# rendeirolab/stainx

Measured on AMD Instinct MI355X. Metric: megapixels/sec Macenko transform, 64x3x512x512 fp32; max-abs vs torch CPU, higher is better.
Workload: dtype f32; 1 GPU; Macenko reference-mode transform, 64x3x512x512 fp32 per GPU (BASELINE configs[1]); tiles_per_gpu=64, height=512, width=512, input_batches_rotated=2, parallelism=tiles sharded over 1 GPU(s), no collective

## Files before the change

### stainx_amd/csrc/macenko.hip

```cpp
#include "common.hpp"

#include <algorithm>
#include <atomic>
#include <type_traits>
#include <cstdlib>

namespace sx {
namespace macenko {

constexpr int kSample = 4096;
constexpr int kMinCap = 8192;
constexpr int kChunk = 16384;
template <typename T> struct PackOf { static constexpr int n = 16 / (int)sizeof(T); };
constexpr int kSlots = 4;
constexpr int kMoments = 20;
constexpr int kPartial = 10;
constexpr int kShortList = 512;
constexpr int kGroupThreads = 1024;
constexpr int kKeys = kSample / kGroupThreads;
constexpr int kPrefetchHist = 8;
constexpr int kPrefetchCand = 8;
static_assert(kKeys * kGroupThreads == kSample && kPrefetchCand * kGroupThreads <= kMinCap, "per-tile stage geometry");

constexpr float kBeta = 0.15f;
// ... 49 lines not shown
    int recon_chunk, recon_blocks;
    int fast;
    int chunk;
    int vec_width;
    int no_tie;
    int out_code;
    int two_pass;
    int prior_units;
    unsigned prior_step_q16;
    uint32_t cap2;
    uint32_t seg_cap;
    uint32_t over_cap;
    int n_seg;
    int spec_fail;
    float spec_kw, spec_eff_far, spec_eff_near, spec_rot, spec_sigmas, spec_sigmas_conc, spec_tscale;
    int fused;
    int dense;
    uint32_t fused_cap;
    int fused_items;
    uint32_t code_epoch;
    const float* aug_alpha;
    const float* aug_beta;
    int own_basis;
};

static Geometry make_geometry(int64_t n_tiles, int64_t pixels, int pooled) {
    Geometry g{};
    g.n_tiles = n_tiles;
    g.pixels = pixels;
    g.blocks_per_tile = (int)((pixels + kChunk - 1) / kChunk);
    g.pooled = pooled;
    g.sample_stride = 1;
    g.cap = (uint32_t)kMinCap;
    g.chunk = kChunk;
    g.vec_width = 1;
    return g;
}

constexpr int kCompact = 32768;
struct alignas(256) PoolState {
    uint32_t hist[2][2][256];
    uint32_t below[kSlots], ncand[kSlots];
    uint32_t compact_n[kSlots];
    uint32_t rank_in_bin[kSlots], range[kSlots][2];
    uint32_t ok[kSlots], overflow;
    uint32_t status;
// ... 313 lines not shown
            return raw_value<T>(v);
        } else if constexpr (sizeof(T) == 4) {
            T v;
            __builtin_memcpy(&v, &w[k][e], 4);
            return raw_value<T>(v);
        } else {
            T v;
            __builtin_memcpy(&v, &w[k][2 * e], 8);
            return raw_value<T>(v);
        }
    }
};

template <int W>
__device__ __forceinline__ void store_codes(const Geometry& g, const Workspace& ws, int64_t tile, int64_t p, const uint32_t (&word)[3][W]) {
    static_assert(W == 1 || W == 2, "four or eight codes per plane");
#pragma unroll
    for (int c = 0; c < 3; ++c) {
        uint8_t* dst = ws.codes + ((size_t)tile * 3 + c) * g.pixels + p;
        if constexpr (W == 1) *reinterpret_cast<uint32_t*>(dst) = word[c][0]; else *reinterpret_cast<uint2*>(dst) = make_uint2(word[c][0], word[c][1]);
    }
}
template <typename T, int V, bool kInter, class Table>
__device__ __forceinline__ void code_quad(const PixelPacks<T, V, kInter>& u, int i0, const LevelTables<T>& tb, const Table& ct, const Geometry& g, const Workspace& ws, int64_t tile, float (&od_quad)[4][3], uint32_t (&word)[3][V / 4]) {
    static_assert((V == 4 || V == 8) && !kInter, "a pack's codes are one or two 32-bit words of a plane");
    constexpr int kCodeCopies = Table::copies;
    uint32_t differ = 0u;
    const int copy = (int)(threadIdx.x % kCodeCopies);
#pragma unroll
    for (int c = 0; c < 3; ++c) {
        uint32_t w = 0u;
#pragma unroll
        for (int ii = 0; ii < 4; ++ii) {
            const float x = u.value(c, i0 + ii);
            const uint32_t k = __float_as_uint(fmaf(x, 255.0f, 8388608.0f)) & 0xFFu;
            const uint2 entry = ct.e[k * kCodeCopies + copy];
            differ |= entry.x ^ __float_as_uint(x);
            od_quad[ii][c] = __uint_as_float(entry.y);
            w |= k << (8 * ii);
        }
        word[c][i0 / 4] = w;
    }
    if (__builtin_expect(__builtin_amdgcn_ballot_w64(differ != 0u) != 0ull, 0)) {
#pragma unroll
        for (int ii = 0; ii < 4; ++ii)
#pragma unroll
            for (int c = 0; c < 3; ++c) {
                float x = u.value(c, i0 + ii);
                asm volatile("" : "+v"(x));
                od_quad[ii][c] = od_of<T>(x, tb);
            }
        if (differ != 0u) put(&ws.code_bad[tile], g.code_epoch);
    }
}


template <typename O, int V, bool kInter>
__device__ __forceinline__ void store_pixels(O* __restrict__ dst, int64_t pixels, int64_t p, const O (&res)[3][V]) {
    if constexpr (kInter) {
        O flat[3][V];
#pragma unroll
        for (int i = 0; i < V; ++i)
#pragma unroll
            for (int c = 0; c < 3; ++c) flat[(3 * i + c) / V][(3 * i + c) % V] = res[c][i];
#pragma unroll
        for (int k = 0; k < 3; ++k) store_pack_stream<O, V>(dst + 3 * p + k * V, flat[k]);
    } else {
#pragma unroll
        for (int c = 0; c < 3; ++c) store_pack_stream<O, V>(dst + c * pixels + p, res[c]);
    }
}

template <typename O, int V>
__device__ __forceinline__ void store_pixels_staged(O* __restrict__ dst, int64_t p, const O (&res)[3][V], uint4* __restrict__ stage) {
    static_assert(sizeof(O) * V == 16, "16-byte packs");
    O flat[3][V];
// ... 2312 lines not shown
    hipLaunchKernelGGL((plane_kernel<T>), dim3(n_groups), dim3(kGroupThreads), 0, stream, images, g, ws, allow_fallback);
    hipLaunchKernelGGL((bracket_kernel<T, V, false, kInter>), dim3(grid_b), dim3(kStreamThreads), 0, stream, images, g, ws);
    if (g.spread) {
        hipLaunchKernelGGL(pool_reduce_kernel, dim3((unsigned)g.n_tiles), dim3(512), 0, stream, g, ws, 0);
        hipLaunchKernelGGL(pool_gather_kernel, dim3((unsigned)g.n_tiles), dim3(kGroupThreads), 0, stream, g, ws, 0);
        hipLaunchKernelGGL((stain_kernel<T, true>), dim3(1), dim3(kGroupThreads), 0, stream, images, g, ws);
    } else {
        hipLaunchKernelGGL((stain_kernel<T>), dim3(n_groups), dim3(kGroupThreads), 0, stream, images, g, ws);
    }
    if (g.own_basis) return check_launch("macenko estimate");
    hipLaunchKernelGGL((bracket_kernel<T, V, true, kInter>), dim3(grid_b), dim3(kStreamThreads), 0, stream, images, g, ws);
    if (g.spread) {
        hipLaunchKernelGGL(pool_reduce_kernel, dim3((unsigned)g.n_tiles), dim3(512), 0, stream, g, ws, 1);
        hipLaunchKernelGGL(pool_gather_kernel, dim3((unsigned)g.n_tiles), dim3(kGroupThreads), 0, stream, g, ws, 1);
        hipLaunchKernelGGL((scale_kernel<T, true>), dim3(1), dim3(kGroupThreads), 0, stream, images, g, ws, tmc, he_out, max_c_out);
    } else {
        hipLaunchKernelGGL((scale_kernel<T>), dim3(n_groups), dim3(kGroupThreads), 0, stream, images, g, ws, tmc, he_out, max_c_out);
    }
    return check_launch("macenko estimate");
}

template <typename T, int V, bool kInter = false>
static int run_two_pass(const T* images, const Geometry& g, const Workspace& ws, const float* tmc, hipStream_t stream, void* key_scratch = nullptr) {
    const unsigned n = (unsigned)g.n_tiles, grid = (unsigned)(g.n_tiles * g.blocks_per_tile);
#ifndef SX_DIAG
    if constexpr (V == 1) {
        return fail(SX_ERR_BAD_ARG, "the two-pass form needs 16-byte aligned tiles of whole packs");
    } else {
        if (!g.dense) return fail(SX_ERR_BAD_ARG, "the two-pass form serves tiles of up to 512 x 512 pixels in this build");
        hipLaunchKernelGGL((prior_kernel<T, true, kInter>), dim3(n), dim3(kGroupThreads), 0, stream, images, g, ws);
        hipLaunchKernelGGL((pass_a_kernel<T, V, kInter, true>), dim3(grid), dim3(kStreamThreads), 0, stream, images, g, ws);
        hipLaunchKernelGGL((estimate_stage_kernel<T, true>), dim3(2 * n), dim3(kGroupThreads), 0, stream, images, g, ws, tmc, static_cast<uint32_t*>(key_scratch));
        return check_launch("macenko two-pass estimate");
    }
#else
    const bool quads = (g.pixels % 4 == 0) && aligned_for(images, 4 * sizeof(T));
    if (quads)
        hipLaunchKernelGGL((prior_kernel<T, true, kInter>), dim3(n), dim3(kGroupThreads), 0, stream, images, g, ws);
    else
        hipLaunchKernelGGL((prior_kernel<T, false, kInter>), dim3(n), dim3(kGroupThreads), 0, stream, images, g, ws);
    if (g.dense) {
        hipLaunchKernelGGL((pass_a_kernel<T, V, kInter, true>), dim3(grid), dim3(kStreamThreads), 0, stream, images, g, ws);
        hipLaunchKernelGGL((estimate_stage_kernel<T, true>), dim3(2 * n), dim3(kGroupThreads), 0, stream, images, g, ws, tmc, static_cast<uint32_t*>(key_scratch));
    } else {
        hipLaunchKernelGGL((pass_a_kernel<T, V, kInter>), dim3(grid), dim3(kStreamThreads), 0, stream, images, g, ws);
        hipLaunchKernelGGL((estimate_stage_kernel<T>), dim3(2 * n), dim3(kGroupThreads), 0, stream, images, g, ws, tmc, static_cast<uint32_t*>(key_scratch));
    }
    return check_launch("macenko two-pass estimate");
#endif
}

#ifdef SX_DIAG
template <typename T, typename O, int V>
static int run_fused(const T* images, O* out, const Geometry& g, const Workspace& ws, const float* sm, const float* tmc, bool unit, hipStream_t stream) {
    const unsigned n = (unsigned)g.n_tiles, units = (unsigned)(2 * g.fused_items) + 2u * n;
    hipLaunchKernelGGL((prior_kernel<T, true, false>), dim3(n), dim3(kGroupThreads), 0, stream, images, g, ws);
    if (unit)
        hipLaunchKernelGGL((fused_kernel<T, O, V, true>), dim3(units), dim3(kStreamThreads), 0, stream, images, out, g, ws, sm, tmc);
    else
        hipLaunchKernelGGL((fused_kernel<T, O, V, false>), dim3(units), dim3(kStreamThreads), 0, stream, images, out, g, ws, sm, tmc);
    return check_launch("macenko fused transform");
// ... 17 lines not shown
    }
    if (rc != SX_OK) return rc;
    constexpr int VR = V == 1 ? 1 : ((int)(16 / sizeof(O)) < V ? (int)(16 / sizeof(O)) : V);
    Geometry gr = g;
    unsigned items_r = items;
    if (!g.recon_chunk && !g.fine_chunk && V > 1 && g.n_tiles * g.pixels >= (1ll << 22)) {
        gr.recon_chunk = kStreamThreads * VR;
        gr.recon_blocks = (int)((g.pixels + gr.recon_chunk - 1) / gr.recon_chunk);
        items_r = (unsigned)(g.n_tiles * gr.recon_blocks);
    }
    if (g.aug_alpha) {
        if (unit)
            hipLaunchKernelGGL((reconstruct_kernel<T, O, VR, true, kInter, true>), dim3(items_r), dim3(kStreamThreads), 0, stream, images, out, gr, ws, sm);
        else
            hipLaunchKernelGGL((reconstruct_kernel<T, O, VR, false, kInter, true>), dim3(items_r), dim3(kStreamThreads), 0, stream, images, out, gr, ws, sm);
    } else if (unit) {
        hipLaunchKernelGGL((reconstruct_kernel<T, O, VR, true, kInter>), dim3(items_r), dim3(kStreamThreads), 0, stream, images, out, gr, ws, sm);
    } else {
        hipLaunchKernelGGL((reconstruct_kernel<T, O, VR, false, kInter>), dim3(items_r), dim3(kStreamThreads), 0, stream, images, out, gr, ws, sm);
    }
    return check_launch("macenko reconstruct");
}

#ifdef SX_DIAG
static int device_cus() {
    static int cached[64] = {0};
    int dev = 0;
    if (hipGetDevice(&dev) != hipSuccess || dev < 0 || dev >= 64) return 256;
    if (cached[dev] == 0) {
        int n = 0;
        if (hipDeviceGetAttribute(&n, hipDeviceAttributeMultiprocessorCount, dev) != hipSuccess || n <= 0) n = 256;
        cached[dev] = n;
    }
    return cached[dev];
}
static int elem_bytes(int dtype) { return dtype == SX_U8 ? 1 : (dtype == SX_F16 || dtype == SX_BF16) ? 2 : dtype == SX_F32 ? 4 : 8; }
static bool resident_able(int dtype, int64_t n, int64_t pixels, unsigned flags) {
    if (dtype != SX_U8 && dtype != SX_F16 && dtype != SX_BF16 && dtype != SX_F32) return false;
    if (flags & (SX_MACENKO_SAMPLED | SX_MACENKO_CHANNELS_LAST | SX_MACENKO_OUT_BF16 | SX_MACENKO_OUT_F16)) return false;
    const int64_t pack = 16 / elem_bytes(dtype);
    if (pixels % pack != 0 || pixels < 1024) return false;
    const int64_t items = (pixels + kChunk - 1) / kChunk, group = (items + kResQuads - 1) / kResQuads;
    return group <= kResMaxGroup && group <= device_cus() && n >= 1;
}
static ResGeom resident_geometry(int dtype, int64_t n, int64_t pixels, bool unit) {
    Geometry g = make_geometry(n, pixels, 0);
    g.vec = 1;
    g.vec_width = 16 / elem_bytes(dtype);
    set_chunk(g, false);
    ResGeom rg{};
    rg.n_tiles = n;
    rg.pixels = pixels;
    rg.items = g.blocks_per_tile;
    rg.chunk = g.chunk;
    rg.group = (rg.items + kResQuads - 1) / kResQuads;
    const int cus = device_cus();
    int fit = std::max(cus / rg.group, 1);
    if (fit >= 8 && n >= 8) {
// ... 71 lines not shown
        g.spec_rot = kSpecRot;
        g.spec_sigmas = kSpecSigmas;
        g.spec_sigmas_conc = kSpecSigmasConc;
        g.spec_tscale = kSpecThresholdScale;
#ifdef SX_STAMPS
        auto knob = [](const char* name, float& v) { if (const char* e = std::getenv(name)) v = (float)std::atof(e); };
        knob("SX_SPEC_KW", g.spec_kw);
        knob("SX_SPEC_EFF_FAR", g.spec_eff_far);
        knob("SX_SPEC_EFF_NEAR", g.spec_eff_near);
        knob("SX_SPEC_ROT", g.spec_rot);
        knob("SX_SPEC_SIGMAS", g.spec_sigmas);
        knob("SX_SPEC_SIGMAS_CONC", g.spec_sigmas_conc);
        knob("SX_SPEC_TSCALE", g.spec_tscale);
#endif
        g.fused_cap = g.fused ? fused_cap_for(g.pixels) : dense_cap_for(g.pixels);
        g.fused_items = (int)(g.n_tiles * g.blocks_per_tile);
        g.cap2 = cap2_for(g.pixels);
        g.n_seg = even_items_size(g.pixels) ? g.blocks_per_tile * (kStreamThreads / kWave) : two_pass_segments(g.pixels);
        g.seg_cap = seg_cap_for(g.pixels);
        g.over_cap = over_cap_for(g.pixels);
        const int64_t n_sectors = g.pixels / 16;
        g.prior_units = (int)std::min<int64_t>(std::max<int64_t>(n_sectors / 4, std::min<int64_t>(n_sectors, 64)), kPriorUnitsMax);
        g.prior_step_q16 = (unsigned)((n_sectors << 16) / g.prior_units);
    }
    if (!g.fused) set_fine_chunk(g, vec ? W : 1);
#ifdef SX_STAMPS
    if (const char* e = std::getenv("SX_RECON_CHUNK")) {
        const int64_t c = std::atoll(e);
        if (c > 0 && !g.fused && c % ((int64_t)kStreamThreads * (vec ? W : 1)) == 0) {
            g.recon_chunk = (int)c;
            g.recon_blocks = (int)((g.pixels + c - 1) / c);
        }
    }
#endif
    const T* in = static_cast<const T*>(images);
    if constexpr (sizeof(T) == 1) {
        if (u8_half) {
#define SX_RUN_HALF(O)                                                                                                                                          \
    return g.interleaved ? (vec ? run_transform<T, O, W, true>(in, static_cast<O*>(out), g, ws, sm, tmc, unit, stream)                                          \
                                : run_transform<T, O, 1, true>(in, static_cast<O*>(out), g, ws, sm, tmc, unit, stream))                                         \
                         : (vec ? run_transform<T, O, W>(in, static_cast<O*>(out), g, ws, sm, tmc, unit, stream)                                                \
                                : run_transform<T, O, 1>(in, static_cast<O*>(out), g, ws, sm, tmc, unit, stream));
            if (g.out_code == SX_BF16) {
                SX_RUN_HALF(__hip_bfloat16)
            } else {
                SX_RUN_HALF(__half)
// ... 934 lines not shown
```

### stainx_amd/csrc/macenko_twopass.hpp

```cpp
#pragma once

namespace sx {
namespace macenko {

constexpr int kPriorSweeps = 4;
constexpr int kPriorUnitsMax = kGroupThreads / 4 * kPriorSweeps;
constexpr int kQueue2 = 512;
constexpr float kSpecSigmasConc = 5.0f, kSpecThresholdScale = 1.0f;
constexpr float kSpecSigmas = 5.0f;
constexpr float kSpecEffFar = 2.0f, kSpecEffNear = 1.0f;
__device__ __forceinline__ float spec_eff(const Geometry& g) { return g.prior_step_q16 >= (8u << 16) ? g.spec_eff_far : g.spec_eff_near; }
constexpr float kSpecKw = 0.10f, kSpecKx = 1.3e-3f;
constexpr float kSpecRot = 0.30f;
constexpr uint32_t kSpecSlow = 1u, kSpecHazard = 2u;
constexpr int kMaxSegments = 256;

constexpr int kRowBelowA = 0, kRowAboveA = 1, kRowBelowB = 2, kRowAboveB = 3, kRowConc = 4, kRowW = 8;
struct alignas(128) PriorRecord {
    float a0[3], a1[3], an[3];
    float rows[16][4];
    float kw, kx;
    float cmax[4];
    int32_t mode;
    int32_t min_first;
    uint32_t open;
};

struct alignas(64) FusedTile {
    uint32_t a_done;
    uint32_t s_done;
    uint32_t ncand[kSlots];
    uint32_t pad[10];
};
constexpr int kXcds = 8;
struct alignas(64) FusedQueue {
    uint32_t ticket;
    uint32_t pad[15];
};
struct FusedSched {
    FusedQueue queue[kXcds];
};
static_assert(sizeof(FusedTile) == kFusedTileBytes && sizeof(FusedSched) <= kFusedSchedBytes, "workspace layout");


typedef unsigned int sx_u4 __attribute__((ext_vector_type(4)));
__device__ __forceinline__ uint32_t ld_agent(const uint32_t* p) { return __hip_atomic_load(p, __ATOMIC_RELAXED, __HIP_MEMORY_SCOPE_AGENT); }
__device__ __forceinline__ int32_t ld_agent(const int32_t* p) { return __hip_atomic_load(p, __ATOMIC_RELAXED, __HIP_MEMORY_SCOPE_AGENT); }
__device__ __forceinline__ float ld_agent(const float* p) { return __uint_as_float(__hip_atomic_load(reinterpret_cast<const uint32_t*>(p), __ATOMIC_RELAXED, __HIP_MEMORY_SCOPE_AGENT)); }
__device__ __forceinline__ double ld_agent(const double* p) {
    return __longlong_as_double((long long)__hip_atomic_load(reinterpret_cast<const unsigned long long*>(p), __ATOMIC_RELAXED, __HIP_MEMORY_SCOPE_AGENT));
}
__device__ __forceinline__ void st_agent(uint32_t* p, uint32_t v) { __hip_atomic_store(p, v, __ATOMIC_RELAXED, __HIP_MEMORY_SCOPE_AGENT); }
__device__ __forceinline__ void st_agent(float* p, float v) { __hip_atomic_store(reinterpret_cast<uint32_t*>(p), __float_as_uint(v), __ATOMIC_RELAXED, __HIP_MEMORY_SCOPE_AGENT); }
__device__ __forceinline__ void st_agent(double* p, double v) {
    __hip_atomic_store(reinterpret_cast<unsigned long long*>(p), (unsigned long long)__double_as_longlong(v), __ATOMIC_RELAXED, __HIP_MEMORY_SCOPE_AGENT);
// ... 56 lines not shown
    const int64_t p = have ? ((int64_t)sector * 4 + (tid & 3)) * 4 : (int64_t)(tid & 3) * 4;
    if constexpr (kVec) {
        load_pixels<T, 4, kInter>(img, g.pixels, p, u);
    } else {
#pragma unroll
        for (int i = 0; i < 4; ++i) {
            float v[3][1];
            load_pixels<T, 1, kInter>(img, g.pixels, p + i, v);
#pragma unroll
            for (int c = 0; c < 3; ++c) u[c][i] = v[c][0];
        }
    }
    return have;
}
template <typename T>
__device__ __forceinline__ void prior_densities(const float (&u)[3][4], float (&od)[4][3]) {
#pragma unroll
    for (int i = 0; i < 4; ++i)
#pragma unroll
        for (int c = 0; c < 3; ++c) od[i][c] = optical_density<T>(u[c][i]);
}

template <typename T, bool kVec, bool kInter>
__global__ __launch_bounds__(kGroupThreads) void prior_kernel(const T* __restrict__ images, Geometry g, Workspace ws) {
    __shared__ PriorScratch sh;
    const int tile = blockIdx.x, tid = threadIdx.x, wave = tid / kWave;
    const uint32_t lane = lane_id();
    GroupState& st = ws.state[tile];
    PriorRecord* pr = &ws.prior[tile];
    const T* img = images + (int64_t)tile * 3 * g.pixels;
    SX_STAMP(st, 0);
    if (tid < kSlots) {
        put(&st.ncand[tid], 0u);
        put(&st.below[tid], 0u);
        put(&st.ncand_seen[tid], 0u);
        put(&st.over_count[tid], 0u);
    }
    if (tid < 2) put(&st.phi_pub[tid], 0ull);
    if ((g.fused || g.dense) && tid < (int)(sizeof(FusedTile) / 4)) put(reinterpret_cast<uint32_t*>(&ws.ftile[tile]) + tid, 0u);
    if (g.fused && tile == 0 && tid >= 32 && tid < 32 + kXcds) put(&ws.fsched->queue[tid - 32].ticket, 0u);
    if (tid == 0) {
        put(&st.fell_back, 0u);
        put(&st.spec, 0u);
        sh.n_kept = sh.n_all = sh.hazard = sh.open = sh.r_max = 0;
        sh.cmax[0] = sh.cmax[1] = sh.cmax[2] = sh.cmax[3] = 0;
    }
    for (int i = tid; i < 5 * kPriorBins; i += kGroupThreads) (&sh.hist[0][0])[i] = 0;

    {
        float m[kPartial];
#pragma unroll
        for (int k = 0; k < kPartial; ++k) m[k] = 0.0f;
        float raw[kPriorSweeps][3][4];
        bool have_quad[kPriorSweeps];
#pragma unroll
        for (int s = 0; s < kPriorSweeps; ++s) have_quad[s] = prior_fetch<T, kVec, kInter>(img, g, s, raw[s]);
#pragma unroll
        for (int s = 0; s < kPriorSweeps; ++s) {
            float od[4][3];
            prior_densities<T>(raw[s], od);
            const bool have = have_quad[s];
#pragma unroll
// ... 240 lines not shown
        }
        if (lane < 16 && (lane < (uint32_t)kRowConc || lane >= (uint32_t)kRowW)) {
#pragma unroll
            for (int c = 0; c < 4; ++c) put(&pr->rows[lane][c], __half2float(__float2half_rn(row[c])));
        }
    } else if (wave == 5 && lane == 0) {
#pragma unroll
        for (int i = 0; i < 3; ++i) {
            put(&pr->a0[i], sh.frame[i]);
            put(&pr->a1[i], sh.frame[3 + i]);
            put(&pr->an[i], sh.frame[6 + i]);
        }
        put(&pr->kw, g.spec_kw);
        put(&pr->kx, kSpecKx);
#pragma unroll
        for (int q = 0; q < 4; ++q) put(&pr->cmax[q], __uint_as_float(sh.cmax[q]));
        put(&pr->mode, 0);
        put(&pr->min_first, min_first ? 1 : 0);
        put(&pr->open, sh.open);
    }
    SX_STAMP(st, 7);
}

template <int TPB> struct PassAScratch {
    StatsScratch<TPB> stats;
    uint32_t queue[TPB / kWave][4][kQueue2];
    uint32_t below[2];
};

__device__ __forceinline__ void write_records(const uint32_t (*__restrict__ queue)[kQueue2], uint32_t n, uint32_t (&have)[kSlots], float* __restrict__ cand_tile, const Geometry& g, uint32_t seg_base, uint32_t* __restrict__ over_count) {
    const uint32_t cap2 = g.cap2, seg_cap = g.seg_cap, over_base = (uint32_t)g.n_seg * g.seg_cap;
    for (uint32_t i0 = 0; i0 < n; i0 += kWave) {
        const uint32_t i = i0 + lane_id();
        uint4 rec = make_uint4(0u, 0u, 0u, 0u);
        if (i < n) rec = make_uint4(queue[0][i], queue[1][i], queue[2][i], queue[3][i]);
#pragma unroll
        for (int s = 0; s < kSlots; ++s) {
            const bool has = ((rec.w >> s) & 1u) != 0;
            const uint64_t mask = __builtin_amdgcn_ballot_w64(has);
            const uint32_t count = (uint32_t)__popcll(mask), at = have[s] + rank_in_mask(mask);
            uint32_t idx = seg_base + at;
            bool store = has;
            if (__builtin_expect(have[s] + count > seg_cap, 0)) {
                const uint64_t spilled = __builtin_amdgcn_ballot_w64(has && at >= seg_cap);
                uint32_t base = 0;
                if (lane_id() == 0) base = atomicAdd(&over_count[s], (uint32_t)__popcll(spilled));
// ... 34 lines not shown
    for (int s = 0; s < kSlots; ++s) at0[s] = (uint32_t)__builtin_amdgcn_readlane((int)base, s);
    const auto rsrc = __builtin_amdgcn_make_buffer_rsrc(rec_tile, 0, (int)(kSlots * cap * 16u), 0x00020000);
    for (uint32_t i0 = 0; i0 < n; i0 += kWave) {
        const uint32_t i = i0 + lane;
        sx_u4 rec = {0u, 0u, 0u, 0u};
        uint32_t flags = 0;
        if (i < n) {
            rec[0] = queue[0][i];
            rec[1] = queue[1][i];
            rec[2] = queue[2][i];
            flags = queue[3][i];
        }
#pragma unroll
        for (int s = 0; s < kSlots; ++s) {
            const bool has = ((flags >> s) & 1u) != 0;
            const uint64_t mask = __builtin_amdgcn_ballot_w64(has);
            const uint32_t at = at0[s] + rank_in_mask(mask);
            if (has && at < cap) __builtin_amdgcn_raw_buffer_store_b128(rec, rsrc, (int)(((uint32_t)s * cap + at) * 16u), 0, 16);
            at0[s] += (uint32_t)__popcll(mask);
        }
    }
}

template <typename T, int V, int TPB, bool kInter, bool kFused = false, bool kEmit = false>
__device__ __forceinline__ void pass_a_item(const T* __restrict__ images, const Geometry& g, const Workspace& ws, int64_t tile, int chunk_id, int64_t item, PassAScratch<TPB>* sh, const LevelTables<T>& tb,
                                            const CodeTable<T, 2>* __restrict__ ct = nullptr) {
    const int64_t p_begin = (int64_t)chunk_id * g.chunk;
    const int64_t p_end = min(p_begin + (int64_t)g.chunk, g.pixels);
    const T* img = images + tile * 3 * g.pixels;
    GroupState& st = ws.state[tile];
    const PriorRecord* __restrict__ pr = &ws.prior[tile];
    const int wave = __builtin_amdgcn_readfirstlane((int)(threadIdx.x / kWave));
    const bool speculate = get(&pr->mode) == 0;
    typedef _Float16 half8 __attribute__((ext_vector_type(8)));
    typedef float float16v __attribute__((ext_vector_type(16)));
    half8 test_rows;
    {
        const uint32_t l = lane_id(), r = l & 31u, h = l >> 5, row_half = (r >> 2) & 1u, test = (r & 3u) + 4u * (r >> 3);
        const float4 coef = *reinterpret_cast<const float4*>(&pr->rows[test][0]);
        const bool mine = h == row_half;
        test_rows[0] = (_Float16)(mine ? coef.x : 0.0f);
        test_rows[1] = (_Float16)(mine ? coef.y : 0.0f);
        test_rows[2] = (_Float16)(mine ? coef.z : 0.0f);
        test_rows[3] = (_Float16)(mine ? coef.w : 0.0f);
        test_rows[4] = test_rows[5] = test_rows[6] = test_rows[7] = (_Float16)0.0f;
    }
    const float kw = get(&pr->kw), kx = get(&pr->kx);
    if (threadIdx.x < 2) sh->below[threadIdx.x] = 0;

    constexpr int kShortRun = 32 / V > 0 ? 32 / V : 1;
    double acc[kPartial];
#pragma unroll
    for (int k = 0; k < kPartial; ++k) acc[k] = 0.0;
    float m[kPartial];
#pragma unroll
    for (int k = 0; k < kPartial; ++k) m[k] = 0.0f;

    uint32_t (*queue)[kQueue2] = sh->queue[wave];
    uint32_t n_q = 0, have[kSlots] = {0u, 0u, 0u, 0u}, below_a = 0, below_b = 0;
    float* cand_tile = ws.cand_od + (size_t)tile * kSlots * 3 * g.cap2;
    const uint32_t seg = (uint32_t)chunk_id * (TPB / kWave) + (uint32_t)wave, seg_base = seg * g.seg_cap;
    auto flush = [&]() {
        if constexpr (kFused)
            write_records_fused(queue, n_q, ws.cand_rec + (size_t)tile * kSlots * g.fused_cap, g.fused_cap, ws.ftile[tile].ncand);
        else
            write_records(queue, n_q, have, cand_tile, g, seg_base, st.over_count);
        n_q = 0;
    };

// ... 29 lines not shown
                uint64_t valid[G];
                float16v forms[G];
#pragma unroll
                for (int gi = 0; gi < G; ++gi) {
#pragma unroll
                    for (int c = 0; c < 3; ++c) {
                        if constexpr (kEmit) od[gi][c] = od_quad[(i0 + gi) % 4][c]; else od[gi][c] = od_of<T>(u.value(c, i0 + gi), tb);
                    }
                    const bool sel = od_selected(od[gi], false);
                    valid[gi] = __builtin_amdgcn_ballot_w64(sel) & live_mask;
                    if (__builtin_amdgcn_inverse_ballot_w64(valid[gi])) {
                        const float* o = od[gi];
                        m[0] += 1.0f;
                        m[1] += o[0];
                        m[2] += o[1];
                        m[3] += o[2];
                        m[4] = fmaf(o[0], o[0], m[4]);
                        m[5] = fmaf(o[0], o[1], m[5]);
                        m[6] = fmaf(o[0], o[2], m[6]);
                        m[7] = fmaf(o[1], o[1], m[7]);
                        m[8] = fmaf(o[1], o[2], m[8]);
                        m[9] = fmaf(o[2], o[2], m[9]);
                    }
                    if constexpr (kTests) {
                        typedef __fp16 fp16x2 __attribute__((ext_vector_type(2)));
                        typedef uint32_t uint4v __attribute__((ext_vector_type(4)));
                        const fp16x2 p01 = __builtin_amdgcn_cvt_pkrtz(od[gi][0], od[gi][1]), p2c = __builtin_amdgcn_cvt_pkrtz(od[gi][2], 1.0f);
                        uint4v packed;
                        packed[0] = __builtin_bit_cast(uint32_t, p01);
                        packed[1] = __builtin_bit_cast(uint32_t, p2c);
                        packed[2] = packed[3] = 0u;
                        float16v zero;
#pragma unroll
                        for (int z = 0; z < 16; ++z) zero[z] = 0.0f;
                        forms[gi] = __builtin_amdgcn_mfma_f32_32x32x16_f16(test_rows, __builtin_bit_cast(half8, packed), zero, 0, 0, 0);
                    }
                }
                if constexpr (kTests) {
#pragma unroll
                    for (int gi = 0; gi < G; ++gi) {
                        const float* o = od[gi];
                        const float16v& f = forms[gi];
                        const float mrg = fmaf(kw, fabsf(f[kRowW]), fmaf(kx, fabsf(o[0]) + fabsf(o[1]) + fabsf(o[2]), 1e-6f));
                        const uint64_t lt_a = __builtin_amdgcn_ballot_w64(f[kRowBelowA] < -mrg), gt_a = __builtin_amdgcn_ballot_w64(f[kRowAboveA] > mrg);
                        const uint64_t lt_b = __builtin_amdgcn_ballot_w64(f[kRowBelowB] < -mrg), gt_b = __builtin_amdgcn_ballot_w64(f[kRowAboveB] > mrg);
                        below_a += (uint32_t)__popcll(valid[gi] & lt_a);
                        below_b += (uint32_t)__popcll(valid[gi] & lt_b);
                        const uint64_t c_a = valid[gi] & ~lt_a & ~gt_a, c_b = valid[gi] & ~lt_b & ~gt_b;
                        const uint64_t c_c = live_mask & (__builtin_amdgcn_ballot_w64(f[kRowConc] >= -mrg) | __builtin_amdgcn_ballot_w64(f[kRowConc + 1] >= -mrg));
                        const uint64_t c_d = live_mask & (__builtin_amdgcn_ballot_w64(f[kRowConc + 2] >= -mrg) | __builtin_amdgcn_ballot_w64(f[kRowConc + 3] >= -mrg));
                        const uint64_t any = c_a | c_b | c_c | c_d;
                        if (any) {
                            uint32_t flags = __builtin_amdgcn_inverse_ballot_w64(c_a) ? 1u : 0u;
                            flags |= __builtin_amdgcn_inverse_ballot_w64(c_b) ? 2u : 0u;
                            flags |= __builtin_amdgcn_inverse_ballot_w64(c_c) ? 4u : 0u;
                            flags |= __builtin_amdgcn_inverse_ballot_w64(c_d) ? 8u : 0u;
                            if (__builtin_amdgcn_inverse_ballot_w64(any)) {
                                const uint32_t at = n_q + rank_in_mask(any);
                                queue[0][at] = __float_as_uint(o[0]);
                                queue[1][at] = __float_as_uint(o[1]);
                                queue[2][at] = __float_as_uint(o[2]);
                                queue[3][at] = flags;
                            }
                            n_q += (uint32_t)__popcll(any);
                        }
                        if (__builtin_expect(n_q > (uint32_t)(kQueue2 - kWave), 0)) flush();
                    }
                }
                if constexpr (V > 4) __builtin_amdgcn_sched_barrier(0);
            }
            if (++in_run == kShortRun) {
#pragma unroll
                for (int k = 0; k < kPartial; ++k) {
                    acc[k] += (double)m[k];
                    m[k] = 0.0f;
                }
                in_run = 0;
            }
        }
    };
    if (speculate) sweep(std::true_type{}); else sweep(std::false_type{});
    if (in_run) {
#pragma unroll
        for (int k = 0; k < kPartial; ++k) acc[k] += (double)m[k];
    }

    StatsScratch<TPB>* ss = &sh->stats;
#pragma unroll
    for (int k = 0; k < kPartial; ++k) {
        const double s = wave_total_f64(acc[k]);
// ... 15 lines not shown
    if (threadIdx.x < kPartial) {
        double s = 0.0;
#pragma unroll
        for (int w = 0; w < TPB / kWave; ++w) s += ss->red[w][threadIdx.x];
        if constexpr (kFused) st_agent(&ws.partial[item * kPartial + threadIdx.x], s); else put(&ws.partial[item * kPartial + threadIdx.x], s);
    }
    if (speculate && threadIdx.x == kPartial) {
        if (sh->below[0]) atomicAdd(&st.below[0], sh->below[0]);
        if (sh->below[1]) atomicAdd(&st.below[1], sh->below[1]);
    }
    double kept_total = 0.0;
#pragma unroll
    for (int w = 0; w < TPB / kWave; ++w) kept_total += ss->red[w][0];
    if (__builtin_expect(kept_total < 3.0, 0)) {
        if (!tile_has_three_kept_witnesses<T, TPB, kInter>(img, g.pixels)) {
            stats_item_all_pixels<T, V, TPB, kInter>(img, g.pixels, p_begin, p_end, ws.partial_all + item * kPartial, ss);
            if constexpr (kFused) __builtin_amdgcn_fence(__ATOMIC_RELEASE, "agent");
        }
    }
    if constexpr (kFused) {
        drain_stores();
        __syncthreads();
        if (threadIdx.x == 0) __hip_atomic_fetch_add(&ws.ftile[tile].a_done, 1u, __ATOMIC_RELAXED, __HIP_MEMORY_SCOPE_AGENT);
    }
}

template <typename T, int V, bool kInter = false, bool kDense = false>
__global__ __launch_bounds__(kStreamThreads, (Codable<T, V, kInter>::value ? 4 : 1)) void pass_a_kernel(const T* __restrict__ images, Geometry g, Workspace ws) {
    __shared__ PassAScratch<kStreamThreads> sh;
    __shared__ LevelTables<T> tb;
    tb.fill();
    if constexpr (Codable<T, V, kInter>::value) {
        if (g.code_epoch != 0u) {
            __shared__ CodeTable<T, 2> ct;
            ct.fill();
            pass_a_item<T, V, kStreamThreads, kInter, kDense, true>(images, g, ws, blockIdx.x / g.blocks_per_tile, blockIdx.x % g.blocks_per_tile, blockIdx.x, &sh, tb, &ct);
            return;
        }
    }
    pass_a_item<T, V, kStreamThreads, kInter, kDense>(images, g, ws, blockIdx.x / g.blocks_per_tile, blockIdx.x % g.blocks_per_tile, blockIdx.x, &sh, tb);
}

struct PhiBinSetup {
    float inv[9];
    float dir[2][2];
};
struct alignas(128) SlotScratch {
    TileScratch t;
    uint32_t keys[kLdsKeys];
    float vecs[6], pinv[6], he[6];
    double check[8];
    uint32_t lo, hi, n_list, bin, rank_in_bin, result, range_first, range_last, bin_count;
    int ok, use_all;
    unsigned long long n_sel;
    uint32_t seg_prefix[kMaxSegments + 1], seg_total, seg_overflow, over_n;
    uint32_t dense_n;
    uint32_t own_key;
    int partner_ok;
// ... 620 lines not shown
```

Measured before the change: 113,300 megapixels/s.

## Overlap early pass-A chunks with the prior kernel on idle CUs

Extra workgroups are added to the prior kernel. They run the coding and moment statistics for the first few chunks of each tile, using CUs that would otherwise sit idle while the per-tile prior is computed. Pass A skips chunks already completed early. It also launches extra units that apply the speculative MFMA tests to those chunks by reading the stored codes back. The number of early chunks is chosen so the total prior grid fits within the device CU count. This adds LDS union scratch, extra code reads for the test units, and coordination through early_done epoch flags.

```diff
diff --git a/stainx_amd/csrc/macenko.hip b/stainx_amd/csrc/macenko.hip
--- a/stainx_amd/csrc/macenko.hip
+++ b/stainx_amd/csrc/macenko.hip
@@ -95,6 +95,7 @@
     const float* aug_alpha;
     const float* aug_beta;
     int own_basis;
+    int early;
 };
 
 static Geometry make_geometry(int64_t n_tiles, int64_t pixels, int pooled) {
@@ -454,7 +455,8 @@
     }
 }
 template <typename T, int V, bool kInter, class Table>
-__device__ __forceinline__ void code_quad(const PixelPacks<T, V, kInter>& u, int i0, const LevelTables<T>& tb, const Table& ct, const Geometry& g, const Workspace& ws, int64_t tile, float (&od_quad)[4][3], uint32_t (&word)[3][V / 4]) {
+__device__ __forceinline__ void code_quad(const PixelPacks<T, V, kInter>& u, int i0, const LevelTables<T>& tb, const Table& ct, const Geometry& g, const Workspace& ws, int64_t tile, float (&od_quad)[4][3], uint32_t (&word)[3][V / 4],
+                                          uint32_t* not_level = nullptr) {
     static_assert((V == 4 || V == 8) && !kInter, "a pack's codes are one or two 32-bit words of a plane");
     constexpr int kCodeCopies = Table::copies;
     uint32_t differ = 0u;
@@ -484,6 +486,7 @@
             }
         if (differ != 0u) put(&ws.code_bad[tile], g.code_epoch);
     }
+    if (not_level) *not_level |= differ;
 }
 
 
@@ -2842,13 +2845,14 @@
 
 template <typename T, int V, bool kInter = false>
 static int run_two_pass(const T* images, const Geometry& g, const Workspace& ws, const float* tmc, hipStream_t stream, void* key_scratch = nullptr) {
-    const unsigned n = (unsigned)g.n_tiles, grid = (unsigned)(g.n_tiles * g.blocks_per_tile);
+    const unsigned n = (unsigned)g.n_tiles, grid = (unsigned)(g.n_tiles * (g.blocks_per_tile + (g.early > 0 ? early_units_per_tile(g) : 0)));
+    const unsigned n_prior = n + (unsigned)((g.n_tiles * g.early + 1) / 2);
 #ifndef SX_DIAG
     if constexpr (V == 1) {
         return fail(SX_ERR_BAD_ARG, "the two-pass form needs 16-byte aligned tiles of whole packs");
     } else {
         if (!g.dense) return fail(SX_ERR_BAD_ARG, "the two-pass form serves tiles of up to 512 x 512 pixels in this build");
-        hipLaunchKernelGGL((prior_kernel<T, true, kInter>), dim3(n), dim3(kGroupThreads), 0, stream, images, g, ws);
+        hipLaunchKernelGGL((prior_kernel<T, true, kInter>), dim3(n_prior), dim3(kGroupThreads), 0, stream, images, g, ws);
         hipLaunchKernelGGL((pass_a_kernel<T, V, kInter, true>), dim3(grid), dim3(kStreamThreads), 0, stream, images, g, ws);
         hipLaunchKernelGGL((estimate_stage_kernel<T, true>), dim3(2 * n), dim3(kGroupThreads), 0, stream, images, g, ws, tmc, static_cast<uint32_t*>(key_scratch));
         return check_launch("macenko two-pass estimate");
@@ -2856,7 +2860,7 @@
 #else
     const bool quads = (g.pixels % 4 == 0) && aligned_for(images, 4 * sizeof(T));
     if (quads)
-        hipLaunchKernelGGL((prior_kernel<T, true, kInter>), dim3(n), dim3(kGroupThreads), 0, stream, images, g, ws);
+        hipLaunchKernelGGL((prior_kernel<T, true, kInter>), dim3(n_prior), dim3(kGroupThreads), 0, stream, images, g, ws);
     else
         hipLaunchKernelGGL((prior_kernel<T, false, kInter>), dim3(n), dim3(kGroupThreads), 0, stream, images, g, ws);
     if (g.dense) {
@@ -2920,7 +2924,6 @@
     return check_launch("macenko reconstruct");
 }
 
-#ifdef SX_DIAG
 static int device_cus() {
     static int cached[64] = {0};
     int dev = 0;
@@ -2932,6 +2935,7 @@
     }
     return cached[dev];
 }
+#ifdef SX_DIAG
 static int elem_bytes(int dtype) { return dtype == SX_U8 ? 1 : (dtype == SX_F16 || dtype == SX_BF16) ? 2 : dtype == SX_F32 ? 4 : 8; }
 static bool resident_able(int dtype, int64_t n, int64_t pixels, unsigned flags) {
     if (dtype != SX_U8 && dtype != SX_F16 && dtype != SX_BF16 && dtype != SX_F32) return false;
@@ -3049,6 +3053,15 @@
         const int64_t n_sectors = g.pixels / 16;
         g.prior_units = (int)std::min<int64_t>(std::max<int64_t>(n_sectors / 4, std::min<int64_t>(n_sectors, 64)), kPriorUnitsMax);
         g.prior_step_q16 = (unsigned)((n_sectors << 16) / g.prior_units);
+    }
+    g.early = 0;
+    if (g.two_pass && g.dense && g.code_epoch != 0u && (g.chunk % 8) == 0) {
+        int e = std::min(kEarlyMax, 3 * g.blocks_per_tile / 8);
+        while (e > 0 && g.n_tiles + (g.n_tiles * e + 1) / 2 > device_cus()) --e;
+        g.early = e;
+#ifdef SX_DIAG
+        if (const char* v = std::getenv("SX_EARLY_ITEMS")) g.early = std::max(0, std::min(std::atoi(v), std::min(kEarlyMax, g.blocks_per_tile - 1)));
+#endif
     }
     if (!g.fused) set_fine_chunk(g, vec ? W : 1);
 #ifdef SX_STAMPS
diff --git a/stainx_amd/csrc/macenko_twopass.hpp b/stainx_amd/csrc/macenko_twopass.hpp
--- a/stainx_amd/csrc/macenko_twopass.hpp
+++ b/stainx_amd/csrc/macenko_twopass.hpp
@@ -13,6 +13,7 @@
 constexpr float kSpecKw = 0.10f, kSpecKx = 1.3e-3f;
 constexpr float kSpecRot = 0.30f;
 constexpr uint32_t kSpecSlow = 1u, kSpecHazard = 2u;
+constexpr int kEarlyMax = 8;
 constexpr int kMaxSegments = 256;
 
 constexpr int kRowBelowA = 0, kRowAboveA = 1, kRowBelowB = 2, kRowAboveB = 3, kRowConc = 4, kRowW = 8;
@@ -30,7 +31,8 @@
     uint32_t a_done;
     uint32_t s_done;
     uint32_t ncand[kSlots];
-    uint32_t pad[10];
+    uint32_t early_done[kEarlyMax];
+    uint32_t pad[10 - kEarlyMax];
 };
 constexpr int kXcds = 8;
 struct alignas(64) FusedQueue {
@@ -133,8 +135,8 @@
 }
 
 template <typename T, bool kVec, bool kInter>
-__global__ __launch_bounds__(kGroupThreads) void prior_kernel(const T* __restrict__ images, Geometry g, Workspace ws) {
-    __shared__ PriorScratch sh;
+__device__ __forceinline__ void prior_tile(const T* __restrict__ images, const Geometry& g, const Workspace& ws, PriorScratch* shp) {
+    PriorScratch& sh = *shp;
     const int tile = blockIdx.x, tid = threadIdx.x, wave = tid / kWave;
     const uint32_t lane = lane_id();
     GroupState& st = ws.state[tile];
@@ -148,7 +150,7 @@
         put(&st.over_count[tid], 0u);
     }
     if (tid < 2) put(&st.phi_pub[tid], 0ull);
-    if ((g.fused || g.dense) && tid < (int)(sizeof(FusedTile) / 4)) put(reinterpret_cast<uint32_t*>(&ws.ftile[tile]) + tid, 0u);
+    if ((g.fused || g.dense) && tid < (int)(offsetof(FusedTile, early_done) / 4)) put(reinterpret_cast<uint32_t*>(&ws.ftile[tile]) + tid, 0u);
     if (g.fused && tile == 0 && tid >= 32 && tid < 32 + kXcds) put(&ws.fsched->queue[tid - 32].ticket, 0u);
     if (tid == 0) {
         put(&st.fell_back, 0u);
@@ -435,6 +437,115 @@
     SX_STAMP(st, 7);
 }
 
+template <typename T> struct EarlyScratch {
+    CodeTable<T, 2> ct;
+    double run[2][kPartial][kStreamThreads];
+    double red[2][kStreamThreads / kWave][kPartial];
+    uint32_t not_level[2];
+};
+template <typename T>
+__device__ __forceinline__ void early_items(const T* __restrict__ images, const Geometry& g, const Workspace& ws, EarlyScratch<T>* sh) {
+    constexpr int V = 4, TPB = kStreamThreads, kShortRun = 32 / V;
+    static_assert(kGroupThreads == 4 * TPB && kChunk <= 2 * kShortRun * TPB * V, "two items per workgroup, two runs per item");
+    LevelTables<T> tb;
+    if (threadIdx.x < 2) sh->not_level[threadIdx.x] = 0u;
+    sh->ct.fill();
+    const int which = (int)threadIdx.x / (2 * TPB), half = ((int)threadIdx.x / TPB) & 1, qt = (int)threadIdx.x % TPB;
+    const int qwave = __builtin_amdgcn_readfirstlane(qt / kWave);
+    const int64_t idx = 2 * ((int64_t)blockIdx.x - g.n_tiles) + which;
+    const bool have_item = idx < g.n_tiles * g.early;
+    const int64_t tile = have_item ? idx / g.early : 0;
+    const int chunk_id = have_item ? (int)(idx % g.early) : 0;
+    const int64_t p_begin = (int64_t)chunk_id * g.chunk, p_end = min(p_begin + (int64_t)g.chunk, g.pixels);
+    const T* img = images + tile * 3 * g.pixels;
+    const int n_sweeps = have_item ? (int)((p_end - p_begin + TPB * V - 1) / (TPB * V)) : 0;
+    const int s_begin = half * kShortRun, s_end = min(s_begin + kShortRun, n_sweeps);
+
+    float m[kPartial];
+#pragma unroll
+    for (int k = 0; k < kPartial; ++k) m[k] = 0.0f;
+    uint32_t not_level = 0u;
+    {
+        const int64_t mine = (int64_t)qt * V;
+        int64_t base_p = p_begin + (int64_t)s_begin * TPB * V;
+        PixelPacks<T, V, false> next;
+        next.clear();
+        if (s_begin < s_end && base_p + mine < p_end) next.load(img, g.pixels, base_p + mine);
+        for (int s = s_begin; s < s_end; ++s, base_p += (int64_t)TPB * V) {
+            const bool live = base_p + mine < p_end;
+            const PixelPacks<T, V, false> u = next;
+            const int64_t p_next = base_p + (int64_t)TPB * V + mine;
+            if (s + 1 < s_end && p_next < p_end) next.load(img, g.pixels, p_next);
+            if (live) {
+                float od_quad[4][3];
+                uint32_t word[3][1];
+                code_quad(u, 0, tb, sh->ct, g, ws, tile, od_quad, word, &not_level);
+                store_codes<1>(g, ws, tile, base_p + mine, word);
+#pragma unroll
+                for (int i = 0; i < V; ++i) {
+                    const float* o = od_quad[i];
+                    if (od_selected(o, false)) {
+                        m[0] += 1.0f;
+                        m[1] += o[0];
+                        m[2] += o[1];
+                        m[3] += o[2];
+                        m[4] = fmaf(o[0], o[0], m[4]);
+                        m[5] = fmaf(o[0], o[1], m[5]);
+                        m[6] = fmaf(o[0], o[2], m[6]);
+                        m[7] = fmaf(o[1], o[1], m[7]);
+                        m[8] = fmaf(o[1], o[2], m[8]);
+                        m[9] = fmaf(o[2], o[2], m[9]);
+                    }
+                }
+            }
+        }
+    }
+    if (half == 1) {
+#pragma unroll
+        for (int k = 0; k < kPartial; ++k) sh->run[which][k][qt] = (double)m[k];
+    }
+    if (not_level != 0u) sh->not_level[which] = 1u;
+    __syncthreads();
+    if (half == 0) {
+#pragma unroll
+        for (int k = 0; k < kPartial; ++k) {
+            const double acc = (double)m[k] + sh->run[which][k][qt];
+            const double s = wave_total_f64(acc);
+            if (lane_id() == kWave - 1) sh->red[which][qwave][k] = s;
+        }
+    }
+    __syncthreads();
+    if (half == 0 && have_item && qt <= kPartial) {
+        double kept_total = 0.0;
+#pragma unroll
+        for (int w = 0; w < TPB / kWave; ++w) kept_total += sh->red[which][w][0];
+        const bool done = !(kept_total < 3.0) && sh->not_level[which] == 0u;
+        if (qt < kPartial) {
+            double s = 0.0;
+#pragma unroll
+            for (int w = 0; w < TPB / kWave; ++w) s += sh->red[which][w][qt];
+            if (done) put(&ws.partial[(tile * g.blocks_per_tile + chunk_id) * kPartial + qt], s);
+        } else {
+            put(&ws.ftile[tile].early_done[chunk_id], done ? g.code_epoch : 0u);
+        }
+    }
+}
+
+template <typename T, bool kVec, bool kInter>
+__global__ __launch_bounds__(kGroupThreads) void prior_kernel(const T* __restrict__ images, Geometry g, Workspace ws) {
+    constexpr bool kEarly = kVec && Codable<T, 4, kInter>::value;
+    if constexpr (kEarly) {
+        __shared__ union Scratch {
+            PriorScratch prior;
+            EarlyScratch<T> early;
+        } sh;
+        if ((int64_t)blockIdx.x < g.n_tiles) prior_tile<T, kVec, kInter>(images, g, ws, &sh.prior); else early_items<T>(images, g, ws, &sh.early);
+    } else {
+        __shared__ PriorScratch sh;
+        prior_tile<T, kVec, kInter>(images, g, ws, &sh);
+    }
+}
+
 template <int TPB> struct PassAScratch {
     StatsScratch<TPB> stats;
     uint32_t queue[TPB / kWave][4][kQueue2];
@@ -515,6 +626,62 @@
     }
 }
 
+typedef _Float16 half8 __attribute__((ext_vector_type(8)));
+typedef float float16v __attribute__((ext_vector_type(16)));
+__device__ __forceinline__ half8 load_test_rows(const PriorRecord* __restrict__ pr) {
+    half8 test_rows;
+    const uint32_t l = lane_id(), r = l & 31u, h = l >> 5, row_half = (r >> 2) & 1u, test = (r & 3u) + 4u * (r >> 3);
+    const float4 coef = *reinterpret_cast<const float4*>(&pr->rows[test][0]);
+    const bool mine = h == row_half;
+    test_rows[0] = (_Float16)(mine ? coef.x : 0.0f);
+    test_rows[1] = (_Float16)(mine ? coef.y : 0.0f);
+    test_rows[2] = (_Float16)(mine ? coef.z : 0.0f);
+    test_rows[3] = (_Float16)(mine ? coef.w : 0.0f);
+    test_rows[4] = test_rows[5] = test_rows[6] = test_rows[7] = (_Float16)0.0f;
+    return test_rows;
+}
+__device__ __forceinline__ float16v test_forms(const half8& test_rows, const float* o) {
+    typedef __fp16 fp16x2 __attribute__((ext_vector_type(2)));
+    typedef uint32_t uint4v __attribute__((ext_vector_type(4)));
+    const fp16x2 p01 = __builtin_amdgcn_cvt_pkrtz(o[0], o[1]), p2c = __builtin_amdgcn_cvt_pkrtz(o[2], 1.0f);
+    uint4v packed;
+    packed[0] = __builtin_bit_cast(uint32_t, p01);
+    packed[1] = __builtin_bit_cast(uint32_t, p2c);
+    packed[2] = packed[3] = 0u;
+    float16v zero;
+#pragma unroll
+    for (int z = 0; z < 16; ++z) zero[z] = 0.0f;
+    return __builtin_amdgcn_mfma_f32_32x32x16_f16(test_rows, __builtin_bit_cast(half8, packed), zero, 0, 0, 0);
+}
+template <class Flush>
+__device__ __forceinline__ void judge_pixel(const float* o, const float16v& f, uint64_t valid, uint64_t live_mask, float kw, float kx, uint32_t& below_a, uint32_t& below_b,
+                                            uint32_t (*queue)[kQueue2], uint32_t& n_q, Flush& flush) {
+    const float mrg = fmaf(kw, fabsf(f[kRowW]), fmaf(kx, fabsf(o[0]) + fabsf(o[1]) + fabsf(o[2]), 1e-6f));
+    const uint64_t lt_a = __builtin_amdgcn_ballot_w64(f[kRowBelowA] < -mrg), gt_a = __builtin_amdgcn_ballot_w64(f[kRowAboveA] > mrg);
+    const uint64_t lt_b = __builtin_amdgcn_ballot_w64(f[kRowBelowB] < -mrg), gt_b = __builtin_amdgcn_ballot_w64(f[kRowAboveB] > mrg);
+    below_a += (uint32_t)__popcll(valid & lt_a);
+    below_b += (uint32_t)__popcll(valid & lt_b);
+    const uint64_t c_a = valid & ~lt_a & ~gt_a, c_b = valid & ~lt_b & ~gt_b;
+    const uint64_t c_c = live_mask & (__builtin_amdgcn_ballot_w64(f[kRowConc] >= -mrg) | __builtin_amdgcn_ballot_w64(f[kRowConc + 1] >= -mrg));
+    const uint64_t c_d = live_mask & (__builtin_amdgcn_ballot_w64(f[kRowConc + 2] >= -mrg) | __builtin_amdgcn_ballot_w64(f[kRowConc + 3] >= -mrg));
+    const uint64_t any = c_a | c_b | c_c | c_d;
+    if (any) {
+        uint32_t flags = __builtin_amdgcn_inverse_ballot_w64(c_a) ? 1u : 0u;
+        flags |= __builtin_amdgcn_inverse_ballot_w64(c_b) ? 2u : 0u;
+        flags |= __builtin_amdgcn_inverse_ballot_w64(c_c) ? 4u : 0u;
+        flags |= __builtin_amdgcn_inverse_ballot_w64(c_d) ? 8u : 0u;
+        if (__builtin_amdgcn_inverse_ballot_w64(any)) {
+            const uint32_t at = n_q + rank_in_mask(any);
+            queue[0][at] = __float_as_uint(o[0]);
+            queue[1][at] = __float_as_uint(o[1]);
+            queue[2][at] = __float_as_uint(o[2]);
+            queue[3][at] = flags;
+        }
+        n_q += (uint32_t)__popcll(any);
+    }
+    if (__builtin_expect(n_q > (uint32_t)(kQueue2 - kWave), 0)) flush();
+}
+
 template <typename T, int V, int TPB, bool kInter, bool kFused = false, bool kEmit = false>
 __device__ __forceinline__ void pass_a_item(const T* __restrict__ images, const Geometry& g, const Workspace& ws, int64_t tile, int chunk_id, int64_t item, PassAScratch<TPB>* sh, const LevelTables<T>& tb,
                                             const CodeTable<T, 2>* __restrict__ ct = nullptr) {
@@ -525,19 +692,7 @@
     const PriorRecord* __restrict__ pr = &ws.prior[tile];
     const int wave = __builtin_amdgcn_readfirstlane((int)(threadIdx.x / kWave));
     const bool speculate = get(&pr->mode) == 0;
-    typedef _Float16 half8 __attribute__((ext_vector_type(8)));
-    typedef float float16v __attribute__((ext_vector_type(16)));
-    half8 test_rows;
-    {
-        const uint32_t l = lane_id(), r = l & 31u, h = l >> 5, row_half = (r >> 2) & 1u, test = (r & 3u) + 4u * (r >> 3);
-        const float4 coef = *reinterpret_cast<const float4*>(&pr->rows[test][0]);
-        const bool mine = h == row_half;
-        test_rows[0] = (_Float16)(mine ? coef.x : 0.0f);
-        test_rows[1] = (_Float16)(mine ? coef.y : 0.0f);
-        test_rows[2] = (_Float16)(mine ? coef.z : 0.0f);
-        test_rows[3] = (_Float16)(mine ? coef.w : 0.0f);
-        test_rows[4] = test_rows[5] = test_rows[6] = test_rows[7] = (_Float16)0.0f;
-    }
+    const half8 test_rows = load_test_rows(pr);
     const float kw = get(&pr->kw), kx = get(&pr->kx);
     if (threadIdx.x < 2) sh->below[threadIdx.x] = 0;
 
@@ -613,50 +768,11 @@
                         m[8] = fmaf(o[1], o[2], m[8]);
                         m[9] = fmaf(o[2], o[2], m[9]);
                     }
-                    if constexpr (kTests) {
-                        typedef __fp16 fp16x2 __attribute__((ext_vector_type(2)));
-                        typedef uint32_t uint4v __attribute__((ext_vector_type(4)));
-                        const fp16x2 p01 = __builtin_amdgcn_cvt_pkrtz(od[gi][0], od[gi][1]), p2c = __builtin_amdgcn_cvt_pkrtz(od[gi][2], 1.0f);
-                        uint4v packed;
-                        packed[0] = __builtin_bit_cast(uint32_t, p01);
-                        packed[1] = __builtin_bit_cast(uint32_t, p2c);
-                        packed[2] = packed[3] = 0u;
-                        float16v zero;
-#pragma unroll
-                        for (int z = 0; z < 16; ++z) zero[z] = 0.0f;
-                        forms[gi] = __builtin_amdgcn_mfma_f32_32x32x16_f16(test_rows, __builtin_bit_cast(half8, packed), zero, 0, 0, 0);
-                    }
+                    if constexpr (kTests) forms[gi] = test_forms(test_rows, od[gi]);
                 }
                 if constexpr (kTests) {
 #pragma unroll
-                    for (int gi = 0; gi < G; ++gi) {
-                        const float* o = od[gi];
-                        const float16v& f = forms[gi];
-                        const float mrg = fmaf(kw, fabsf(f[kRowW]), fmaf(kx, fabsf(o[0]) + fabsf(o[1]) + fabsf(o[2]), 1e-6f));
-                        const uint64_t lt_a = __builtin_amdgcn_ballot_w64(f[kRowBelowA] < -mrg), gt_a = __builtin_amdgcn_ballot_w64(f[kRowAboveA] > mrg);
-                        const uint64_t lt_b = __builtin_amdgcn_ballot_w64(f[kRowBelowB] < -mrg), gt_b = __builtin_amdgcn_ballot_w64(f[kRowAboveB] > mrg);
-                        below_a += (uint32_t)__popcll(valid[gi] & lt_a);
-                        below_b += (uint32_t)__popcll(valid[gi] & lt_b);
-                        const uint64_t c_a = valid[gi] & ~lt_a & ~gt_a, c_b = valid[gi] & ~lt_b & ~gt_b;
-                        const uint64_t c_c = live_mask & (__builtin_amdgcn_ballot_w64(f[kRowConc] >= -mrg) | __builtin_amdgcn_ballot_w64(f[kRowConc + 1] >= -mrg));
-                        const uint64_t c_d = live_mask & (__builtin_amdgcn_ballot_w64(f[kRowConc + 2] >= -mrg) | __builtin_amdgcn_ballot_w64(f[kRowConc + 3] >= -mrg));
-                        const uint64_t any = c_a | c_b | c_c | c_d;
-                        if (any) {
-                            uint32_t flags = __builtin_amdgcn_inverse_ballot_w64(c_a) ? 1u : 0u;
-                            flags |= __builtin_amdgcn_inverse_ballot_w64(c_b) ? 2u : 0u;
-                            flags |= __builtin_amdgcn_inverse_ballot_w64(c_c) ? 4u : 0u;
-                            flags |= __builtin_amdgcn_inverse_ballot_w64(c_d) ? 8u : 0u;
-                            if (__builtin_amdgcn_inverse_ballot_w64(any)) {
-                                const uint32_t at = n_q + rank_in_mask(any);
-                                queue[0][at] = __float_as_uint(o[0]);
-                                queue[1][at] = __float_as_uint(o[1]);
-                                queue[2][at] = __float_as_uint(o[2]);
-                                queue[3][at] = flags;
-                            }
-                            n_q += (uint32_t)__popcll(any);
-                        }
-                        if (__builtin_expect(n_q > (uint32_t)(kQueue2 - kWave), 0)) flush();
-                    }
+                    for (int gi = 0; gi < G; ++gi) judge_pixel(od[gi], forms[gi], valid[gi], live_mask, kw, kx, below_a, below_b, queue, n_q, flush);
                 }
                 if constexpr (V > 4) __builtin_amdgcn_sched_barrier(0);
             }
@@ -718,6 +834,55 @@
         drain_stores();
         __syncthreads();
         if (threadIdx.x == 0) __hip_atomic_fetch_add(&ws.ftile[tile].a_done, 1u, __ATOMIC_RELAXED, __HIP_MEMORY_SCOPE_AGENT);
+    }
+}
+
+constexpr int kEarlyUnitPacks = 2048, kEarlyPack = 4;
+__host__ __device__ inline int early_units_per_tile(const Geometry& g) { return (g.early * (g.chunk / kEarlyPack) + kEarlyUnitPacks - 1) / kEarlyUnitPacks; }
+template <typename T, int TPB>
+__device__ __forceinline__ void early_tests_unit(const Geometry& g, const Workspace& ws, uint32_t tile, uint32_t unit, PassAScratch<TPB>* sh, const CodeTable<T, 2>* __restrict__ ct) {
+    const PriorRecord* __restrict__ pr = &ws.prior[tile];
+    if (get(&pr->mode) != 0) return;
+    const int wave = __builtin_amdgcn_readfirstlane((int)(threadIdx.x / kWave));
+    const half8 test_rows = load_test_rows(pr);
+    const float kw = get(&pr->kw), kx = get(&pr->kx);
+    uint32_t (*queue)[kQueue2] = sh->queue[wave];
+    uint32_t n_q = 0, below_a = 0, below_b = 0;
+    auto flush = [&]() {
+        write_records_fused(queue, n_q, ws.cand_rec + (size_t)tile * kSlots * g.fused_cap, g.fused_cap, ws.ftile[tile].ncand);
+        n_q = 0;
+    };
+    constexpr int VS = kEarlyPack;
+    const uint32_t item_packs = (uint32_t)g.chunk / VS, n_packs = (uint32_t)g.early * item_packs;
+    const uint32_t first = unit * kEarlyUnitPacks, last = min(first + (uint32_t)kEarlyUnitPacks, n_packs);
+    uint32_t done = 0;
+    for (int e = 0; e < g.early; ++e) done |= get(&ws.ftile[tile].early_done[e]) == g.code_epoch ? 1u << e : 0u;
+    const int copy = (int)(threadIdx.x % 2);
+    const uint8_t* codes = ws.codes + (size_t)tile * 3 * g.pixels;
+    for (uint32_t k0 = first; k0 < last; k0 += TPB) {
+        const uint32_t k = k0 + threadIdx.x, kk = k < last ? k : first;
+        const bool live = k < last && ((done >> (kk / item_packs)) & 1u) != 0;
+        uint64_t live_mask = __builtin_amdgcn_ballot_w64(live);
+        asm volatile("" : "+s"(live_mask));
+        if (live_mask == 0ull) continue;
+        uint32_t w[3];
+#pragma unroll
+        for (int c = 0; c < 3; ++c) w[c] = get(reinterpret_cast<const uint32_t*>(codes + (size_t)c * g.pixels + (size_t)kk * VS));
+#pragma unroll
+        for (int i = 0; i < VS; ++i) {
+            float o[3];
+#pragma unroll
+            for (int c = 0; c < 3; ++c) o[c] = __uint_as_float(ct->e[((w[c] >> (8 * i)) & 0xFFu) * 2u + copy].y);
+            const uint64_t valid = __builtin_amdgcn_ballot_w64(od_selected(o, false)) & live_mask;
+            const float16v f = test_forms(test_rows, o);
+            judge_pixel(o, f, valid, live_mask, kw, kx, below_a, below_b, queue, n_q, flush);
+        }
+    }
+    flush();
+    if (lane_id() == 0) {
+        GroupState& st = ws.state[tile];
+        if (below_a) atomicAdd(&st.below[0], below_a);
+        if (below_b) atomicAdd(&st.below[1], below_b);
     }
 }
 
@@ -730,6 +895,22 @@
         if (g.code_epoch != 0u) {
             __shared__ CodeTable<T, 2> ct;
             ct.fill();
+            if constexpr (kDense) {
+                if (g.early > 0) {
+                    const uint32_t blk = blockIdx.x, late = (uint32_t)(g.blocks_per_tile - g.early), n_late = (uint32_t)g.n_tiles * late, n_items = (uint32_t)g.n_tiles * (uint32_t)g.blocks_per_tile;
+                    if (blk >= n_items) {
+                        const uint32_t per_tile = (uint32_t)early_units_per_tile(g), u = blk - n_items;
+                        early_tests_unit<T, kStreamThreads>(g, ws, u / per_tile, u % per_tile, &sh, &ct);
+                        return;
+                    }
+                    const bool is_late = blk < n_late;
+                    const uint32_t num = is_late ? blk : blk - n_late, den = is_late ? late : (uint32_t)g.early;
+                    const uint32_t tile = num / den, chunk_id = num - tile * den + (is_late ? (uint32_t)g.early : 0u);
+                    if (!is_late && get(&ws.ftile[tile].early_done[chunk_id]) == g.code_epoch) return;
+                    pass_a_item<T, V, kStreamThreads, kInter, kDense, true>(images, g, ws, tile, (int)chunk_id, tile * (uint32_t)g.blocks_per_tile + chunk_id, &sh, tb, &ct);
+                    return;
+                }
+            }
             pass_a_item<T, V, kStreamThreads, kInter, kDense, true>(images, g, ws, blockIdx.x / g.blocks_per_tile, blockIdx.x % g.blocks_per_tile, blockIdx.x, &sh, tb, &ct);
             return;
         }
```

Result: slower. 107,500 megapixels/s (-5.1%).
